# tianhao-stan-wu/LLA-MPC

Measured on AMD Instinct MI355X. Metric: model-rollouts/sec (N_models x H steps) per control tick; wall-clock per plan() call, higher is better.
Workload: dtype f64

## Files before the change

### lla-mpc_amd/csrc/final_dev.hpp

```cpp
#pragma once
#include "dev_stamps.hpp"
#include "dev_wave.hpp"
#include "lookback_dev.hpp"

namespace llampc {

__device__ __forceinline__ bool ent_less(const Ent& x, const Ent& y) {
  return less_nan_last(x.v, x.i, y.v, y.i);
}

template <typename E>
__device__ __forceinline__ E merge_path_at(const E* A, const E* B, int K, int k) {
  int lo = 0, hi = k;
  while (lo < hi) {
    const int i = (lo + hi) >> 1;
    if (less_nan_last(A[i].v, A[i].i, B[k - i - 1].v, B[k - i - 1].i)) lo = i + 1;
    else hi = i;
  }
  const int i = lo, j = k - lo;
  return (less_nan_last(A[i].v, A[i].i, B[j].v, B[j].i)) ? A[i] : B[j];
}

template <typename E>
__device__ __forceinline__ E* tree_merge(E* buf0, E* buf1, int L, int K) {
  E* src = buf0;
  E* dst = buf1;
  while (L > 1) {
    const int P = (L + 1) >> 1;
    for (int t = threadIdx.x; t < P * K; t += blockDim.x) {
      const int p = t / K, k = t - p * K;
      const E* A = src + (size_t)(2 * p) * K;
      dst[t] = (2 * p + 1 < L) ? merge_path_at(A, A + K, K, k) : A[k];
    }
    __syncthreads();
    E* tmp = src;
    src = dst;
    dst = tmp;
    L = P;
  }
  return src;
}

struct CtlSel {
  uint64_t* tag;
  uint32_t seq;
  uint32_t* ids;
  double* dr;
  double* df;
  double* xv;
  int32_t* xlate;
};

template <int SEL = 0>
__device__ __forceinline__ void lb_final(const FinalLaunch& f, unsigned char* smem, const CtlSel* cs = nullptr) {
  STAMP(0);
  const int tid = threadIdx.x;
  const int L = f.nb_lb;
  const int La = f.nb_lb * kWaves;
  const int K = f.K, M = L * K;
  uint64_t* thr = reinterpret_cast<uint64_t*>(smem + kScratchBytes);
  uint64_t* key = thr + 2;
  double* val = reinterpret_cast<double*>(key + M);
  uint64_t* hk = reinterpret_cast<uint64_t*>(val + M);
  uint64_t* ck = hk + L;
  Ent* am = reinterpret_cast<Ent*>(ck + M);
  uint32_t* id = reinterpret_cast<uint32_t*>(am + La);
  uint32_t* hid = id + M;
  uint32_t* cid = hid + L;
  int* ce = reinterpret_cast<int*>(cid + M);
  int* top = ce + M;
  int* cnt = top + LLAMPC_KMAX;
  auto local = [&](int64_t gi) { return gi == kNoIndex ? kNoLocal : (uint32_t)(gi - f.goff); };
  for (int e = tid; e < M; e += kBlock) {
    const double v = ld_wt(&f.tk_val[e]);
    const uint32_t l = local(ld_wt(&f.tk_idx[e]));
    const uint64_t k = l == kNoLocal ? ~0ull : order_key(v);
    const uint32_t i = l == kNoLocal ? kNoModelId + (uint32_t)e : l;
    key[e] = k;
    val[e] = v;
    id[e] = i;
    if (e % K == 0) {
      hk[e / K] = k;
      hid[e / K] = i;
    }
  }
  for (int b = tid; b < La; b += kBlock) am[b] = Ent{ld_wt(&f.am_val[b]), ld_wt(&f.am_idx[b])};
  if (tid == 0) {
    *cnt = 0;
    thr[0] = ~0ull;
    thr[1] = 0xFFFFFFFFull;
  }
  __syncthreads();
  STAMP(1);
  auto lt = [](uint64_t ka, uint32_t ia, uint64_t kb, uint32_t ib) {
    return (int)(ka < kb) | ((int)(ka == kb) & (int)(ia < ib));
  };
  if (L >= K) {
    for (int h = tid; h < L; h += kBlock) {
      const uint64_t mk = hk[h];
      const uint32_t mi = hid[h];
      int r = 0;
#pragma unroll 8
      for (int j = 0; j < L; ++j) r += lt(hk[j], hid[j], mk, mi);
      if (r == K - 1) {
        thr[0] = mk;
        thr[1] = mi;
      }
    }
    __syncthreads();
  }
  STAMP(6);
  const uint64_t tk = thr[0];
  const uint32_t ti = (uint32_t)thr[1];
  for (int e = tid; e < M; e += kBlock) {
    const uint64_t k = key[e];
    const uint32_t i = id[e];
    if (!lt(tk, ti, k, i)) {
      const int slot = atomicAdd(cnt, 1);
      ck[slot] = k;
      cid[slot] = i;
      ce[slot] = e;
    }
  }
  __syncthreads();
  STAMP(7);
  const int c = *cnt;
  for (int q = tid; q < c; q += kBlock) {
    const uint64_t mk = ck[q];
    const uint32_t mi = cid[q];
    int r = 0;
#pragma unroll 8
    for (int j = 0; j < c; ++j) r += lt(ck[j], cid[j], mk, mi);
    if (r < K) top[r] = ce[q];
  }
  __syncthreads();
  if (tid >= 64) return;
  const int lane = tid;
  double v = f.nan_first ? __builtin_inf() : __builtin_nan("");
  uint32_t li = kNoLocal;
  for (int b = lane; b < La; b += 64) {
    const double bv = am[b].v;
    const uint32_t bl = local(am[b].i);
    const bool t = (int)(bl != kNoLocal) &
                   (int)(f.nan_first ? less_bf<1>(bv, bl, v, li) : less_bf<0>(bv, bl, v, li));
    v = t ? bv : v;
    li = t ? bl : li;
  }
  if (f.nan_first) wave_pick_nf(v, li);
  else wave_pick_nl(v, li);
  double kv = __builtin_nan("");
  uint32_t kl = kNoLocal;
  if (lane < K) {
    const int e = top[lane];
    kl = id[e] >= kNoModelId ? kNoLocal : id[e];
    kv = val[e];
  }
  STAMP(2);
  if constexpr (SEL == 2) {
    if (lane < K) {
      cs->ids[lane] = kl;
      cs->xv[lane] = kv;
    }
    if (lane == 0) {
      cs->ids[K] = li;
      cs->xv[K] = v;
    }
    return;
  }
  if constexpr (SEL == 1) {
    if (lane < K) {
      cs->ids[lane] = kl;
      st_wt(&cs->tag[lane], tag_word(cs->seq, kl));
    }
    if (lane == 0) {
      cs->ids[K] = li;
      st_wt(&cs->tag[K], tag_word(cs->seq, li));
    }
  }
  llampc_plan_out* o = f.out;
  if (lane < LLAMPC_KMAX) {
    const int k = lane;
    if (k < K && kl != kNoLocal) {
      st_wt(&o->topk[k], f.goff + (int64_t)kl);
      st_wt(&o->topk_val[k], kv);
      st_wt(&o->topk_Df[k], f.params[2 * f.n + kl]);
      st_wt(&o->topk_Dr[k], f.params[5 * f.n + kl]);
    } else {
      const double nan = __builtin_nan("");
      st_wt(&o->topk[k], (int64_t)-1);
      st_wt(&o->topk_val[k], nan);
      st_wt(&o->topk_Df[k], nan);
      st_wt(&o->topk_Dr[k], nan);
    }
  }
  if (lane == 0) {
    st_wt(&o->lb_best, li == kNoLocal ? (int64_t)-1 : f.goff + (int64_t)li);
    st_wt(&o->lb_best_val, li == kNoLocal ? __builtin_nan("") : v);
  }
  if constexpr (SEL == 1) {
    if (lane < K) {
      const bool have = kl != kNoLocal;
      cs->dr[lane] = have ? f.params[5 * f.n + kl] : __builtin_nan("");
      cs->df[lane] = have ? f.params[2 * f.n + kl] : __builtin_nan("");
    }
  }
}

__device__ __forceinline__ void final_write(const FinalLaunch& f, bool lb, int64_t sel, bool owned,
                                            int32_t kcand, double kcost, int32_t scand,
                                            double scost, double lav, int64_t lai, int nf,
                                            int status = 0) {
  const int tid = threadIdx.x;
  llampc_plan_out* o = f.out;
  const double nan = __builtin_nan("");
  if (tid < LLAMPC_KMAX) {
    const int k = tid;
    if (!lb) {
      st_wt(&o->topk[k], (int64_t)-1);
      st_wt(&o->topk_val[k], nan);
      st_wt(&o->topk_Df[k], nan);
      st_wt(&o->topk_Dr[k], nan);
    }
    st_wt(&o->topk_cand[k], kcand);
    st_wt(&o->topk_cost[k], kcost);
  }
  if (tid == 0) {
    if (!lb) {
      st_wt(&o->lb_best, (int64_t)-1);
      st_wt(&o->lb_best_val, nan);
    }
    st_wt(&o->window_count, f.window_count);
    st_wt(&o->window_full, f.full);
    st_wt(&o->K, f.K);
    st_wt(&o->n_nonfinite, nf);
    st_wt(&o->status, status);
    st_wt(&o->sel_model, sel);
    st_wt(&o->sel_owned, (int32_t)owned);
    st_wt(&o->sel_cand, scand);
    st_wt(&o->sel_cost, scost);
    const bool la_ok = f.do_la && lai != kNoIndex;
    st_wt(&o->la_best_model, la_ok ? lai / f.C : (int64_t)-1);
    st_wt(&o->la_best_cand, la_ok ? (int32_t)(lai % f.C) : (int32_t)-1);
    st_wt(&o->la_best_cost, la_ok ? lav : nan);
    __hip_atomic_store(&f.tickets[0], 0u, __ATOMIC_RELAXED, __HIP_MEMORY_SCOPE_AGENT);
    __hip_atomic_store(&f.tickets[1], 0u, __ATOMIC_RELAXED, __HIP_MEMORY_SCOPE_AGENT);
    if (f.wq) __hip_atomic_store(f.wq, (uint64_t)0, __ATOMIC_RELAXED, __HIP_MEMORY_SCOPE_AGENT);
  }
  if (f.host_tag) {
    __threadfence_system();
    __syncthreads();
    if (tid == 0) __hip_atomic_store(f.host_tag, f.host_seq, __ATOMIC_RELAXED, __HIP_MEMORY_SCOPE_SYSTEM);
  }
  STAMP(5);
#ifdef LLAMPC_STAMPS
  if (tid == 0) g_stamp_launch++;
#endif
}

__device__ __forceinline__ void final_select(const FinalLaunch& f, const Scratch& sc) {
  STAMP(3);
  const int tid = threadIdx.x;
  llampc_plan_out* o = f.out;
  const bool lb = f.do_lb && f.full;
  const int64_t idk = (lb && tid < LLAMPC_KMAX) ? ld_wt(&o->topk[tid]) : -1;
  const int64_t lbi = (tid == 0 && lb) ? ld_wt(&o->lb_best) : -1;
  const int64_t sel = lbi >= 0 ? lbi : f.current_model;
  const bool owned = sel >= f.goff && sel < f.goff + f.n;
  const bool have = lb && tid < LLAMPC_KMAX && idk >= 0 && f.do_la;
  int32_t kcand = -1, scand = -1;
  double kcost = __builtin_nan(""), scost = __builtin_nan("");
  if (have) {
    kcand = ld_wt(&f.best_cand[idk - f.goff]);
    kcost = ld_wt(&f.best_cost[idk - f.goff]);
  }
  if (tid == 0 && owned && f.do_la) {
    scand = ld_wt(&f.best_cand[sel - f.goff]);
    scost = ld_wt(&f.best_cost[sel - f.goff]);
  }
  double lav = __builtin_nan("");
  int64_t lai = kNoIndex;
  int nf = 0;
  if (f.do_la) {
    for (int b = tid; b < f.nb_la; b += kBlock) {
      nf += ld_wt(&f.pnf[b]);
      const int64_t pi = ld_wt(&f.pidx[b]);
      const double pv = ld_wt(&f.pv[b]);
      const bool t = (int)(pi != kNoIndex) & (int)less_bf<0>(pv, pi, lav, lai);
      lav = t ? pv : lav;
      lai = t ? pi : lai;
    }
    wave_pick_nl64(lav, lai);
    nf = wave_sum(nf);
    if ((tid & 63) == 0) {
      sc.sv[4 + (tid >> 6)] = lav;
      sc.si[4 + (tid >> 6)] = lai;
      sc.sn[tid >> 6] = nf;
    }
    __syncthreads();
    lav = sc.sv[4];
    lai = sc.si[4];
    nf = sc.sn[0];
#pragma unroll
    for (int w = 1; w < kWaves; ++w) {
      const bool t = (int)(sc.si[4 + w] != kNoIndex) & (int)less_bf<0>(sc.sv[4 + w], sc.si[4 + w], lav, lai);
      lav = t ? sc.sv[4 + w] : lav;
      lai = t ? sc.si[4 + w] : lai;
      nf += sc.sn[w];
    }
  }
  STAMP(4);
  final_write(f, lb, sel, owned, kcand, kcost, scand, scost, lav, lai, nf);
}

constexpr int kPollTimeoutStatus = LLAMPC_STATUS_POLL_TIMEOUT;
__device__ __forceinline__ void final_poll(const FinalLaunch& f, const Scratch& sc) {
  STAMP(3);
  const int tid = threadIdx.x;
  llampc_plan_out* o = f.out;
  const bool lb = f.do_lb && f.full;
  const int64_t idk = (lb && tid < LLAMPC_KMAX) ? ld_wt(&o->topk[tid]) : -1;
  const int64_t lbi = (tid == 0 && lb) ? ld_wt(&o->lb_best) : -1;
  const int64_t sel = lbi >= 0 ? lbi : f.current_model;
  const bool owned = sel >= f.goff && sel < f.goff + f.n;
  const int64_t mk = (lb && tid < LLAMPC_KMAX && idk >= 0) ? idk - f.goff : -1;
  const int64_t ms = (tid == 0 && owned) ? sel - f.goff : -1;
  const int nbt = (f.nb_la + kBlock - 1) / kBlock;
  uint64_t kw[3] = {0, 0, 0}, sw[3] = {0, 0, 0};
  double lav = __builtin_nan("");
  int64_t lai = kNoIndex;
  int nf = 0;
  int status = 0;
  const uint64_t t0 = __builtin_amdgcn_s_memrealtime();
  const uint64_t bound = (uint64_t)(uint32_t)f.poll << 16;
  bool late = false;
  if (mk >= 0) {
    for (;;) {
#pragma unroll
      for (int w = 0; w < 3; ++w) kw[w] = ld_wt(&f.la_tag[w * f.n + mk]);
      if ((int)tag_ok(kw[0], f.seq) & (int)tag_ok(kw[1], f.seq) & (int)tag_ok(kw[2], f.seq)) break;
      if (__builtin_amdgcn_s_memrealtime() - t0 > bound) { late = true; break; }
    }
  }
  if (ms >= 0) {
    for (;;) {
#pragma unroll
      for (int w = 0; w < 3; ++w) sw[w] = ld_wt(&f.la_tag[w * f.n + ms]);
      if ((int)tag_ok(sw[0], f.seq) & (int)tag_ok(sw[1], f.seq) & (int)tag_ok(sw[2], f.seq)) break;
      if (__builtin_amdgcn_s_memrealtime() - t0 > bound) { late = true; break; }
    }
  }
  for (int j = 0; j < nbt; ++j) {
    const int b = tid + j * kBlock;
    if (b < f.nb_la) {
      uint64_t r[5];
      for (;;) {
#pragma unroll
        for (int w = 0; w < 5; ++w) r[w] = ld_wt(&f.blk_tag[5 * (int64_t)b + w]);
        if ((int)tag_ok(r[0], f.seq) & (int)tag_ok(r[1], f.seq) & (int)tag_ok(r[2], f.seq) &
            (int)tag_ok(r[3], f.seq) & (int)tag_ok(r[4], f.seq))
          break;
        if (__builtin_amdgcn_s_memrealtime() - t0 > bound) { late = true; break; }
      }
      const double pv = __longlong_as_double((long long)join_words(r[0], r[1]));
      const int64_t pi = (int64_t)join_words(r[2], r[3]);
      nf += (int)(uint32_t)r[4];
      const bool t = (int)(pi != kNoIndex) & (int)less_bf<0>(pv, pi, lav, lai);
      lav = t ? pv : lav;
      lai = t ? pi : lai;
    }
  }
  unsigned char* late_w = reinterpret_cast<unsigned char*>(sc.sv) + kLateOff;
  const int wlate = __any((int)late);
  int32_t kcand = -1, scand = -1;
  double kcost = __builtin_nan(""), scost = __builtin_nan("");
  if (mk >= 0 && f.do_la) {
    kcost = __longlong_as_double((long long)join_words(kw[0], kw[1]));
    kcand = (int32_t)(uint32_t)kw[2];
  }
  if (ms >= 0 && f.do_la) {
    scost = __longlong_as_double((long long)join_words(sw[0], sw[1]));
    scand = (int32_t)(uint32_t)sw[2];
  }
  wave_pick_nl64(lav, lai);
  nf = wave_sum(nf);
  if ((tid & 63) == 0) {
    sc.sv[4 + (tid >> 6)] = lav;
    sc.si[4 + (tid >> 6)] = lai;
    sc.sn[tid >> 6] = nf;
    late_w[tid >> 6] = (unsigned char)wlate;
  }
  __syncthreads();
  lav = sc.sv[4];
  lai = sc.si[4];
  nf = sc.sn[0];
  int anyl = late_w[0];
#pragma unroll
  for (int w = 1; w < kWaves; ++w) {
    const bool t = (int)(sc.si[4 + w] != kNoIndex) & (int)less_bf<0>(sc.sv[4 + w], sc.si[4 + w], lav, lai);
    lav = t ? sc.sv[4 + w] : lav;
    lai = t ? sc.si[4 + w] : lai;
    nf += sc.sn[w];
    anyl |= late_w[w];
  }
  if (anyl) status = kPollTimeoutStatus;
  STAMP(4);
  final_write(f, lb, sel, owned, kcand, kcost, scand, scost, lav, lai, nf, status);
}

}
```

### lla-mpc_amd/csrc/plan_dev.hpp

```cpp
#pragma once
#include "final_dev.hpp"
#include "lookahead_dev.hpp"
#include "lookback_dev.hpp"
#include "peer_dev.hpp"

namespace llampc {

template <int INTEG, bool STAGE, int LPM, int XM, bool PX = false, int WQ = 0, bool CORR = false>
__device__ __forceinline__ void plan_body(const LookbackLaunch& lb, const LookaheadLaunch& la,
                                          const FinalLaunch& fin, int G, int cpl,
                                          const double* hp = nullptr, double cw = 0.0) {
  extern __shared__ __attribute__((aligned(16))) unsigned char smem[];
  const Scratch sc(smem);
  int* flag = reinterpret_cast<int*>(smem + kFlagOff);
  const bool is_lb = (int)blockIdx.x < fin.nb_lb;
  const int lb_blk = (int)blockIdx.x, la_blk = (int)blockIdx.x - fin.nb_lb;
  if constexpr (wq_threads(WQ) > kBlock) {
    if (is_lb && threadIdx.x >= kBlock) return;
  }
  if (is_lb) {
    lookback_block(lb, lb_blk, sc);
    if (!ticket_last(&fin.tickets[0], (unsigned)fin.nb_lb, flag)) return;
    if (fin.full) {
      lb_final(fin, smem);
      if (fin.host_tag) __threadfence_system();
    }
    if (fin.poll) {
      __syncthreads();
      final_poll(fin, sc);
      if constexpr (PX) peer_finish(fin, smem);
      return;
    }
  } else {
    if constexpr (CORR) lookahead_block<INTEG, STAGE, LPM, XM, WQ, true>(la, la_blk, G, cpl, smem, sc, hp, cw);
    else lookahead_block<INTEG, STAGE, LPM, XM, WQ>(la, la_blk, G, cpl, smem, sc);
    if (fin.poll) return;
    if constexpr (wq_threads(WQ) > kBlock) {
      if (threadIdx.x >= kBlock) return;
    }
  }
  const unsigned expected = (unsigned)fin.nb_la + (fin.nb_lb > 0 ? 1u : 0u);
  if (!ticket_last(&fin.tickets[1], expected, flag)) return;
  final_select(fin, sc);
  if constexpr (PX) peer_finish(fin, smem);
}

constexpr int kArgLa = sizeof(LookbackLaunch), kArgFin = kArgLa + sizeof(LookaheadLaunch);
constexpr int kArgG = kArgFin + sizeof(FinalLaunch), kPlanArgBytes = kArgG + 2 * sizeof(int);
static_assert(sizeof(LookbackLaunch) % 8 == 0 && sizeof(LookaheadLaunch) % 8 == 0 && sizeof(FinalLaunch) % 8 == 0,
              "plan kernel arguments: no padding between the launch structs");

template <int INTEG, bool STAGE, int LPM, int XM, bool PX = false, int WQ = 0>
__global__ __launch_bounds__(wq_threads(WQ)) void plan_kernel(LookbackLaunch lb, LookaheadLaunch la,
                                                      FinalLaunch fin, int G, int cpl) {
  if constexpr (XM || WQ) {
    plan_body<INTEG, STAGE, LPM, XM, PX, WQ>(lb, la, fin, G, cpl);
  } else {
    const KernargPtr kp = touch_kernargs<kPlanArgBytes>();
    plan_body<INTEG, STAGE, LPM, XM, PX, WQ>(kernarg_at<LookbackLaunch>(kp, 0), kernarg_at<LookaheadLaunch>(kp, kArgLa),
                                             kernarg_at<FinalLaunch>(kp, kArgFin), kernarg_at<int>(kp, kArgG),
                                             kernarg_at<int>(kp, kArgG + 4));
  }
}

template <int LPM>
__global__ __launch_bounds__(kBlock) void plan_kernel_inl(LookbackLaunch, LookaheadLaunch, FinalLaunch, int, int,
                                                          InlinePack pk) {
  const KernargPtr kp = touch_kernargs<kPlanArgBytes>();
  LookbackLaunch lb = kernarg_at<LookbackLaunch>(kp, 0);
  LookaheadLaunch la = kernarg_at<LookaheadLaunch>(kp, kArgLa);
  const double* v = pk.v;
  lb.x_prev = v;
  lb.u_prev = v + 6;
  lb.x_now = v + 8;
  la.x0 = v + 8;
  la.uprev = v + 14;
  la.xref = v + 16;
  la.U = v + 16 + 2 * (la.H + 1);
  plan_body<0, true, LPM, 0>(lb, la, kernarg_at<FinalLaunch>(kp, kArgFin), kernarg_at<int>(kp, kArgG),
                             kernarg_at<int>(kp, kArgG + 4));
}

template <int INTEG, bool STAGE, int LPM>
__global__ __launch_bounds__(kBlock) void plan_kernel_corr(LookbackLaunch, LookaheadLaunch, FinalLaunch, int, int,
                                                           PlanCorridor cor) {
  const KernargPtr kp = touch_kernargs<kPlanArgBytes>();
  plan_body<INTEG, STAGE, LPM, 0, false, 0, true>(kernarg_at<LookbackLaunch>(kp, 0), kernarg_at<LookaheadLaunch>(kp, kArgLa),
                                                  kernarg_at<FinalLaunch>(kp, kArgFin), kernarg_at<int>(kp, kArgG),
                                                  kernarg_at<int>(kp, kArgG + 4), cor.hp, cor.weight);
}

template <int INTEG, bool STAGE, int PX, int WQ>
static void launch_plan_wq(const LookbackLaunch& lb, const LookaheadLaunch& la, const FinalLaunch& f,
                           int G, int cpl, size_t lds, hipStream_t s) {
  allow_lds(plan_kernel<INTEG, STAGE, 1, 0, PX, WQ>);
  hipLaunchKernelGGL((plan_kernel<INTEG, STAGE, 1, 0, PX, WQ>), dim3(f.nb_lb + f.nb_la), dim3(wq_threads(WQ)),
                     lds, s, lb, la, f, G, cpl);
}

template <int INTEG, bool STAGE, int LPM>
static void launch_plan_t(const LookbackLaunch& lb, const LookaheadLaunch& la, const FinalLaunch& f,
                          int G, int cpl, size_t lds, hipStream_t s, int wq = 0) {
  if constexpr (INTEG == LLAMPC_RK4 && LPM == 1) {
    if (wq) {
      if constexpr (STAGE) {
        if (wq == 2) {
          if (f.px_G) launch_plan_wq<INTEG, STAGE, 1, 2>(lb, la, f, G, cpl, lds, s);
          else launch_plan_wq<INTEG, STAGE, 0, 2>(lb, la, f, G, cpl, lds, s);
          return;
        }
      }
      if (f.px_G) launch_plan_wq<INTEG, STAGE, 1, 1>(lb, la, f, G, cpl, lds, s);
      else launch_plan_wq<INTEG, STAGE, 0, 1>(lb, la, f, G, cpl, lds, s);
      return;
    }
  }
  if constexpr (INTEG == LLAMPC_RK4) {
    if (f.px_G) {
      allow_lds(plan_kernel<INTEG, STAGE, LPM, 0, true>);
      hipLaunchKernelGGL((plan_kernel<INTEG, STAGE, LPM, 0, true>), dim3(f.nb_lb + f.nb_la), dim3(kBlock), lds,
                         s, lb, la, f, G, cpl);
      return;
    }
  }
  if (la.xref_mode == LLAMPC_XREF_RACELINE) {
    allow_lds(plan_kernel<INTEG, STAGE, LPM, 1>);
    hipLaunchKernelGGL((plan_kernel<INTEG, STAGE, LPM, 1>), dim3(f.nb_lb + f.nb_la), dim3(kBlock), lds, s,
                       lb, la, f, G, cpl);
  } else {
    allow_lds(plan_kernel<INTEG, STAGE, LPM, 0>);
    hipLaunchKernelGGL((plan_kernel<INTEG, STAGE, LPM, 0>), dim3(f.nb_lb + f.nb_la), dim3(kBlock), lds, s,
                       lb, la, f, G, cpl);
  }
}

template <int LPM>
static void launch_plan_inl(const LookbackLaunch& lb, const LookaheadLaunch& la, const FinalLaunch& f,
                            int G, int cpl, size_t lds, hipStream_t s, const InlinePack& pk) {
  allow_lds(plan_kernel_inl<LPM>);
  hipLaunchKernelGGL((plan_kernel_inl<LPM>), dim3(f.nb_lb + f.nb_la), dim3(kBlock), lds, s, lb, la, f,
                     G, cpl, pk);
}

template <int INTEG, int LPM>
void launch_plan_group(const LookbackLaunch& lb, const LookaheadLaunch& la, const FinalLaunch& f, int G,
                       int cpl, bool stage, size_t lds, hipStream_t s, int wq) {
  if (stage) launch_plan_t<INTEG, true, LPM>(lb, la, f, G, cpl, lds, s, wq);
  else launch_plan_t<INTEG, false, LPM>(lb, la, f, G, cpl, lds, s, wq);
}

template <int LPM>
void launch_plan_inline_group(const LookbackLaunch& lb, const LookaheadLaunch& la, const FinalLaunch& f,
                              int G, int cpl, size_t lds, hipStream_t s, const InlinePack& pk) {
  launch_plan_inl<LPM>(lb, la, f, G, cpl, lds, s, pk);
}

template <int INTEG, bool STAGE, int LPM>
static void launch_plan_corr(const LookbackLaunch& lb, const LookaheadLaunch& la, const FinalLaunch& f, int G,
                             int cpl, size_t lds, hipStream_t s, const PlanCorridor& cor) {
  allow_lds(plan_kernel_corr<INTEG, STAGE, LPM>);
  hipLaunchKernelGGL((plan_kernel_corr<INTEG, STAGE, LPM>), dim3(f.nb_lb + f.nb_la), dim3(kBlock), lds, s, lb, la, f,
                     G, cpl, cor);
}

template <int INTEG, int LPM>
void launch_plan_corridor_group(const LookbackLaunch& lb, const LookaheadLaunch& la, const FinalLaunch& f, int G,
                                int cpl, bool stage, size_t lds, hipStream_t s, const PlanCorridor& cor) {
  if (stage) launch_plan_corr<INTEG, true, LPM>(lb, la, f, G, cpl, lds, s, cor);
  else launch_plan_corr<INTEG, false, LPM>(lb, la, f, G, cpl, lds, s, cor);
}

}
```

### lla-mpc_amd/csrc/plan_track_dev.hpp

```cpp
#pragma once
#include "corridor_block_dev.hpp"
#include "ctl_door_dev.hpp"
#include "plan_dev.hpp"

namespace llampc {

#ifdef LLAMPC_STAMPS
static __device__ unsigned long long g_trk_ph[1024][8];
#define TRK_STAMP(slot)                                                                              \
  do {                                                                                               \
    if (threadIdx.x == 0 && blockIdx.x < 1024) g_trk_ph[blockIdx.x][slot] = __builtin_amdgcn_s_memrealtime(); \
  } while (0)
#else
#define TRK_STAMP(slot) LLAMPC_NO_STAMP
#endif

__device__ __forceinline__ void track_corridor_block(const PlanTrack& k, int kk, unsigned char* smem) {
  TRK_STAMP(0);
  const bool valid = k.path_ok != 0 && *k.valid_rd != 0;
  const double nan = __builtin_nan("");
  double px = nan, py = nan, p0x = nan, p0y = nan;
  if (valid) {
    px = k.path_rd[kk];
    py = k.path_rd[kPlanPathStride + kk];
    if (kk == 1) {
      p0x = k.path_rd[0];
      p0y = k.path_rd[kPlanPathStride];
    }
  }
  auto emit = [&](const double* row, double theta) {
    uint64_t* w = k.hp_tag + 12 * (size_t)(kk - 1);
#pragma unroll
    for (int i = 0; i < 6; ++i) {
      const uint64_t b = (uint64_t)__double_as_longlong(row[i]);
      st_wt(&w[2 * i], tag_word(k.seq, (uint32_t)(b >> 32)));
      st_wt(&w[2 * i + 1], tag_word(k.seq, (uint32_t)b));
    }
    double* d = k.dbg;
    d[kk] = px;
    d[kPlanPathStride + kk] = py;
    if (kk == 1) {
      d[0] = p0x;
      d[kPlanPathStride] = p0y;
      *k.dbg_valid = valid;
    }
    double* dh = d + 2 * kPlanPathStride + 6 * (size_t)(kk - 1);
#pragma unroll
    for (int i = 0; i < 6; ++i) dh[i] = row[i];
    d[2 * kPlanPathStride + 6 * LLAMPC_HMAX + (kk - 1)] = theta;
    TRK_STAMP(1);
  };
  if (valid) {
    corridor_block(k.trk, smem, px, py, k.hw, emit);
  } else if (threadIdx.x == 0) {
    const double inf = __builtin_inf();
    const double row[6] = {0.0, 0.0, inf, 0.0, 0.0, inf};
    emit(row, nan);
  }
}

__device__ __forceinline__ int track_poll_hp(const PlanTrack& k, int H, double* shp) {
  uint32_t* hp32 = reinterpret_cast<uint32_t*>(shp);
  int any = 0;
  for (int e = threadIdx.x; e < 12 * H; e += kBlock) {
    int late = 0;
    const uint32_t v = poll_tag(k.hp_tag, e, k.seq, k.poll, late);
    hp32[(e & ~1) | ((e & 1) ^ 1)] = late ? 0u : v;
    any |= late;
  }
  return any;
}

__device__ __forceinline__ void track_stage_write(const LookaheadLaunch& a, double* o, double ua, double dl, double sd,
                                                  double cd, double p0, double p1, const FusedK& fq0) {
  const double d0 = ua - p0, d1 = dl - p1;
  const FusedIn fi = fused_in(fq0, Input{ua, dl, sd, cd});
  o[0] = fi.F0;
  o[1] = fi.F1;
  o[2] = fi.hmsd;
  o[3] = fi.hmcd;
  o[4] = fi.c5a;
  o[5] = dl;
  o[6] = act_term(a.cost, d0, d1);
  o[7] = (!a.cost.enforce || input_feasible(a.cost, ua, dl, d0, d1)) ? 1.0 : 0.0;
}

__device__ __forceinline__ void track_pin_consts(CostK& q, VehK& veh, double& Ts) {
  for (int m = 0; m < 4; ++m) {
    pin_vgpr(q.Q[m]);
    pin_vgpr(q.R[m]);
    pin_vgpr(q.P[m]);
  }
  for (int m = 0; m < 2; ++m) {
    pin_vgpr(q.umin[m]);
    pin_vgpr(q.umax[m]);
    pin_vgpr(q.dmax[m]);
  }
  pin_vgpr(veh.lf);
  pin_vgpr(veh.lr);
  pin_vgpr(veh.mass);
  pin_vgpr(veh.inv_mass);
  pin_vgpr(veh.inv_Iz);
  pin_vgpr(veh.Cm1);
  pin_vgpr(veh.Cm2);
  pin_vgpr(veh.Cr0);
  pin_vgpr(veh.Cr2);
  pin_vgpr(Ts);
}

template <int LPM>
__device__ __forceinline__ void track_model_setup(const VehK& veh, const Tire& t, int sub, double Ts, StageK& sk,
                                                  FusedK& fq) {
  constexpr bool kScaled = scaled_yaw(LPM);
  sk = make_stage<LPM>(veh, t, sub, Ts, Ts * veh.inv_mass);
  if (kScaled) sk.ch[0].lw = sk.ch[0].lw / Ts;
  if (kScaled && LPM == 1) sk.ch[1].lw = sk.ch[1].lw / Ts;
  if (kScaled && LPM == 4 && sub >= 2) {
    sk.ch[0].lw = 0.0;
    sk.ch[0].sg = 0.0;
    sk.ch[0].B = 0.0;
    sk.ch[0].nsB = 0.0;
    sk.Bfw = 0.0;
  }
  fq = make_fused(veh, sk, Ts, kScaled, LPM == 4);
}

template <bool STAGE, int LPM>
__device__ __forceinline__ void track_lookahead_block(const LookaheadLaunch& a, int blk, int G, int cpl,
                                                      unsigned char* smem, const Scratch& sc, const PlanTrack& trk) {
  LA_STAMP(blk, 0);
  TRK_STAMP(0);
  constexpr int BT = kBlock;
  double* sx = reinterpret_cast<double*>(smem + kScratchBytes);
  double* su = sx + 2 * (a.H + 1);
  const int H = a.H, C = a.C;
  double* shp = su + (STAGE ? kStageW * C * H : 0);
  const int sub = threadIdx.x % LPM;
  const int cl = threadIdx.x / LPM;
  const int g = cl & (G - 1);
  const int64_t n = (int64_t)blk * (kBlock / (G * LPM)) + cl / G;
  const bool live = n < a.n;
  Tire t{};
  if (live) t = load_tire(a.params, a.n, n);
  double x0[6];
  CostK q = a.cost;
  VehK veh = a.veh;
  double Ts = a.Ts;
  StageK sk;
  FusedK fq;
  fm::FmK K0;
  double up0, up1;
  {
    const int CH = C * H, tid = (int)threadIdx.x;
    uint32_t zoff;
    asm volatile("v_mov_b32 %0, 0" : "=v"(zoff));
    const double* gx0 = a.x0 + zoff;
    const double* gup = a.uprev + zoff;
    double xv[6];
#pragma unroll
    for (int m = 0; m < 6; ++m) xv[m] = gx0[m];
    const double uv0 = gup[0], uv1 = gup[1];
    const int ex = tid < H ? tid : H;
    const double xr0 = a.xref[ex], xr1 = a.xref[(H + 1) + ex];
    auto stage_load = [&](int e, double& ua, double& dl, double& p0, double& p1) {
      const int ec = e < CH ? e : CH - 1, ep = ec > 0 ? ec - 1 : 0;
      ua = a.U[2 * ec];
      dl = a.U[2 * ec + 1];
      p0 = a.U[2 * ep];
      p1 = a.U[2 * ep + 1];
    };
    double sua = 0.0, sdl = 0.0, sp0 = 0.0, sp1 = 0.0;
    if (STAGE) stage_load(tid, sua, sdl, sp0, sp1);
    K0 = load_la_consts<0, LPM>();
    track_pin_consts(q, veh, Ts);
    track_model_setup<LPM>(veh, t, sub, Ts, sk, fq);
    for (int e = tid; e <= H; e += BT) {
      sx[2 * e] = e == tid ? xr0 : a.xref[e];
      sx[2 * e + 1] = e == tid ? xr1 : a.xref[(H + 1) + e];
    }
#pragma unroll
    for (int m = 0; m < 6; ++m) x0[m] = readfirstlane_d(xv[m]);
    up0 = readfirstlane_d(uv0);
    up1 = readfirstlane_d(uv1);
    if (STAGE) {
      const FusedK fq0 = make_fused(a.veh, make_stage<1>(a.veh, Tire{}, 0), a.Ts, scaled_yaw(LPM));
      auto stage_elem = [&](int e, double ua, double dl, double p0, double p1) {
        const int c = C == 1 ? 0 : e / H, k = e - c * H;
        double sd, cd;
        if (fm::sincos_fast_ok(dl)) fm::sincos_fast(dl, &sd, &cd, K0);
        else LL_SINCOS(dl, &sd, &cd);
        track_stage_write(a, su + kStageW * (k * C + c), ua, dl, sd, cd, k ? p0 : uv0, k ? p1 : uv1, fq0);
      };
      if (tid < CH) stage_elem(tid, sua, sdl, sp0, sp1);
      constexpr int kStageBatch = 4;
      for (int base = tid + BT; base < CH; base += kStageBatch * BT) {
        double ua[kStageBatch], dl[kStageBatch], p0[kStageBatch], p1[kStageBatch];
#pragma unroll
        for (int j = 0; j < kStageBatch; ++j) stage_load(base + j * BT, ua[j], dl[j], p0[j], p1[j]);
#pragma unroll
        for (int j = 0; j < kStageBatch; ++j)
          if (base + j * BT < CH) stage_elem(base + j * BT, ua[j], dl[j], p0[j], p1[j]);
      }
    }
    asm volatile("" ::"v"(xr0), "v"(xr1), "v"(sua), "v"(sdl), "v"(sp0), "v"(sp1));
    TRK_STAMP(1);
    if (track_poll_hp(trk, H, shp)) {
      st_wt(trk.late, trk.seq);
      asm volatile("s_waitcnt vmcnt(0)" ::: "memory");
    }
    TRK_STAMP(2);
    __syncthreads();
  }

  double bv = __builtin_nan("");
  int64_t bc = kNoIndex;
  int nf = 0;
  LA_STAMP(blk, 1);
  constexpr unsigned kRF = STAGE ? kRStage : 0u;
  const double cw = trk.weight;
  if (live) {
    const fm::FmK K = K0;
    for (int j = 0; j < cpl; ++j) {
      const int c = g + j * G;
      if (c >= C) break;
      bool bad = false;
      double J = rollout<0, LPM, kRF | kRFast | kRCorr>(a, c, n, x0, sx, su, veh, t, sk, q, Ts, up0, up1, K, fq, bad,
                                                        nullptr, nullptr, nullptr, 0, nullptr, shp, cw);
      if (LPM == 2) {
        const int bi = bad;
        bad = __builtin_amdgcn_mov_dpp(bi, kPair0, 0xF, 0xF, false) |
              __builtin_amdgcn_mov_dpp(bi, kPair1, 0xF, 0xF, false);
      } else if (LPM == 4) {
        int bi = bad;
        bi |= __builtin_amdgcn_mov_dpp(bi, kQuadX1, 0xF, 0xF, false);
        bi |= __builtin_amdgcn_mov_dpp(bi, kQuadX2, 0xF, 0xF, false);
        bad = bi;
      }
      if (__builtin_expect(__any(bad), 0)) {
        bool unused = false;
        if (bad) J = rollout<0, LPM, kRF | kRCorr>(a, c, n, x0, sx, su, veh, t, sk, q, Ts, up0, up1, K, fq, unused,
                                                   nullptr, nullptr, nullptr, 0, nullptr, shp, cw);
      }
      if (sub == 0) {
        if (a.cost_out) a.cost_out[n * C + c] = J;
        nf += !isfinite(J);
      }
      if (less_nan_last(J, c, bv, bc)) {
        bv = J;
        bc = c;
      }
    }
  }
  LA_STAMP(blk, 2);
  TRK_STAMP(3);
  const int span = G * LPM;
  for (int off = (span < 64 ? span : 64) >> 1; off >= LPM; off >>= 1) {
    const double ov = __shfl_xor(bv, off, 64);
    const int64_t oc = __shfl_xor(bc, off, 64);
    if (less_nan_last(ov, oc, bv, bc)) {
      bv = ov;
      bc = oc;
    }
  }
  int par = 0;
  if (span > 64) {
    double* sv = sc.sv + 4 * par;
    int64_t* si = sc.si + 4 * par;
    par ^= 1;
    if ((threadIdx.x & 63) == 0) {
      sv[threadIdx.x >> 6] = bv;
      si[threadIdx.x >> 6] = bc;
    }
    __syncthreads();
    const int w0 = (int)(threadIdx.x / span) * (span / 64);
    bv = sv[w0];
    bc = si[w0];
    for (int k = 1; k < span / 64; ++k) {
      if (less_nan_last(sv[w0 + k], si[w0 + k], bv, bc)) {
        bv = sv[w0 + k];
        bc = si[w0 + k];
      }
    }
  }
  if (live && g == 0 && sub == 0) {
    if (a.poll) {
      st_wt(&a.la_tag[n], tag_word(a.seq, (uint32_t)(__double_as_longlong(bv) >> 32)));
      st_wt(&a.la_tag[a.n + n], tag_word(a.seq, (uint32_t)__double_as_longlong(bv)));
      st_wt(&a.la_tag[2 * a.n + n], tag_word(a.seq, (uint32_t)(int32_t)bc));
    } else {
      st_wt(&a.best_cand[n], (int32_t)bc);
      st_wt(&a.best_cost[n], bv);
    }
  }
  const int64_t key = (live && bc != kNoIndex && g == 0 && sub == 0) ? (a.goff + n) * C + bc : kNoIndex;
  la_publish(a, blk, sc, par, (key == kNoIndex) ? __builtin_nan("") : bv, key, nf);
  LA_STAMP(blk, 3);
  TRK_STAMP(4);
}

template <bool STAGE, int LPM>
__device__ __forceinline__ void track_path_update(const LookaheadLaunch& a, const FinalLaunch& f, const PlanTrack& trk,
                                                  unsigned char* smem) {
  const int tid = threadIdx.x, H = a.H;
  double* sx = reinterpret_cast<double*>(smem + kScratchBytes);
  double* su = sx + 2 * (H + 1);
  double* shp = su + kStageW * H;
  double* ppos = shp + 6 * H;
  double* sx0 = ppos + 2 * (H + 1);
  double* pcost = sx0 + 6;
  int64_t* psel = reinterpret_cast<int64_t*>(pcost + 1);
  int* pint = reinterpret_cast<int*>(psel + 1);
  __syncthreads();
  if (tid == 0) {
    psel[0] = ld_wt(&f.out->sel_model);
    pint[0] = ld_wt(&f.out->sel_cand);
    pint[1] = ld_wt(&f.out->sel_owned);
    pint[2] = 0;
    *pcost = __builtin_nan("");
  }
  __syncthreads();
  const int64_t sel = psel[0];
  const int cand = pint[0];
  const bool can = pint[1] == 1 && cand >= 0 && cand < a.C && sel >= a.goff && sel < a.goff + a.n;
  if (!can) {
    if (tid == 0) {
      *trk.cost_wr = __builtin_nan("");
      *trk.valid_wr = 0;
    }
    return;
  }
  LookaheadLaunch a1 = a;
  a1.C = 1;
  a1.U = a.U + 2 * (size_t)cand * H;
  const fm::FmK K0 = load_la_consts<0, LPM>();
  for (int e = tid; e <= H; e += kBlock) {
    sx[2 * e] = a.xref[e];
    sx[2 * e + 1] = a.xref[(H + 1) + e];
  }
  if (tid < 6) sx0[tid] = a.x0[tid];
  const double uv0 = a.uprev[0], uv1 = a.uprev[1];
  if (STAGE) {
    const FusedK fq0 = make_fused(a.veh, make_stage<1>(a.veh, Tire{}, 0), a.Ts, scaled_yaw(LPM));
    for (int k = tid; k < H; k += kBlock) {
      const double ua = a1.U[2 * k], dl = a1.U[2 * k + 1];
      const double p0 = k ? a1.U[2 * k - 2] : uv0, p1 = k ? a1.U[2 * k - 1] : uv1;
      double sd, cd;
      if (fm::sincos_fast_ok(dl)) fm::sincos_fast(dl, &sd, &cd, K0);
      else LL_SINCOS(dl, &sd, &cd);
      track_stage_write(a, su + kStageW * k, ua, dl, sd, cd, p0, p1, fq0);
    }
  }
  (void)track_poll_hp(trk, H, shp);
  __syncthreads();
  if (tid < LPM) {
    const int sub = tid;
    const Tire t = load_tire(a.params, a.n, sel - a.goff);
    CostK q = a.cost;
    VehK veh = a.veh;
    double Ts = a.Ts;
    track_pin_consts(q, veh, Ts);
    StageK sk;
    FusedK fq;
    track_model_setup<LPM>(veh, t, sub, Ts, sk, fq);
    double x0[6];
#pragma unroll
    for (int m = 0; m < 6; ++m) x0[m] = sx0[m];
    constexpr unsigned kRF = STAGE ? kRStage : 0u;
    double* dp = sub == 0 ? ppos : nullptr;
    bool bad = false, unused = false;
    double Jw = rollout<0, LPM, kRF | kRFast | kRCorr | kRPos>(a1, 0, sel - a.goff, x0, sx, su, veh, t, sk, q, Ts, uv0, uv1,
                                                               K0, fq, bad, nullptr, nullptr, dp, H + 1, nullptr, shp,
                                                               trk.weight);
    merge_bad<LPM>(bad);
    if (bad)
      Jw = rollout<0, LPM, kRF | kRCorr | kRPos>(a1, 0, sel - a.goff, x0, sx, su, veh, t, sk, q, Ts, uv0, uv1, K0, fq,
                                                 unused, nullptr, nullptr, dp, H + 1, nullptr, shp, trk.weight);
    if (sub == 0) {
      *pcost = Jw;
      pint[2] = (int)(fabs(Jw) <= __DBL_MAX__);
    }
  }
  __syncthreads();
  if (tid < 64) {
    bool ok = pint[2] != 0;
    for (int e = tid; e < 2 * (H + 1); e += 64) {
      const int row = e / (H + 1), j = e - row * (H + 1);
      const double v = ppos[row * (H + 1) + ctl_path_index(j, H)];
      ok = ok && fabs(v) <= __DBL_MAX__;
      trk.path_wr[row * kPlanPathStride + j] = v;
    }
    const int all = __all(ok);
    if (tid == 0) {
      *trk.cost_wr = *pcost;
      *trk.valid_wr = all;
    }
  }
  TRK_STAMP(7);
}

__device__ __forceinline__ void track_finish(const FinalLaunch& f, const PlanTrack& trk) {
  if (threadIdx.x == 0 && ld_wt(trk.late) == trk.seq) st_wt(&f.out->status, (int32_t)kPollTimeoutStatus);
  if (f.host_tag) {
    __threadfence_system();
    __syncthreads();
    if (threadIdx.x == 0) __hip_atomic_store(f.host_tag, f.host_seq, __ATOMIC_RELAXED, __HIP_MEMORY_SCOPE_SYSTEM);
  }
}

template <bool STAGE, int LPM>
__device__ __forceinline__ void plan_track_body(const LookbackLaunch& lb, const LookaheadLaunch& la,
                                                const FinalLaunch& fin, int G, int cpl, const PlanTrack& trk) {
  extern __shared__ __attribute__((aligned(16))) unsigned char smem[];
  const Scratch sc(smem);
  int* flag = reinterpret_cast<int*>(smem + kFlagOff);
  const int blk = (int)blockIdx.x, H = la.H;
  if (blk >= fin.nb_lb && blk < fin.nb_lb + H) {
    track_corridor_block(trk, blk - fin.nb_lb + 1, smem);
    return;
  }
  FinalLaunch fq = fin;
  fq.host_tag = nullptr;
  const bool is_lb = blk < fin.nb_lb;
  if (is_lb) {
    lookback_block(lb, blk, sc);
    if (!ticket_last(&fin.tickets[0], (unsigned)fin.nb_lb, flag)) return;
    if (fin.full) {
      lb_final(fin, smem);
      if (fin.host_tag) __threadfence_system();
    }
    if (fin.poll) {
      __syncthreads();
      TRK_STAMP(5);
      final_poll(fq, sc);
      track_finish(fin, trk);
      TRK_STAMP(6);
      track_path_update<STAGE, LPM>(la, fin, trk, smem);
      return;
    }
  } else {
    track_lookahead_block<STAGE, LPM>(la, blk - fin.nb_lb - H, G, cpl, smem, sc, trk);
    if (fin.poll) return;
  }
  const unsigned expected = (unsigned)fin.nb_la + (fin.nb_lb > 0 ? 1u : 0u);
  if (!ticket_last(&fin.tickets[1], expected, flag)) return;
  TRK_STAMP(5);
  final_select(fq, sc);
  track_finish(fin, trk);
  TRK_STAMP(6);
  track_path_update<STAGE, LPM>(la, fin, trk, smem);
}

constexpr int kArgTrack = kPlanArgBytes;
static_assert(kPlanArgBytes % alignof(PlanTrack) == 0, "the PlanTrack lies right behind (G, cpl)");

template <bool STAGE, int LPM>
__global__ __launch_bounds__(kBlock) void plan_kernel_track(LookbackLaunch, LookaheadLaunch, FinalLaunch, int, int,
                                                            PlanTrack) {
  const KernargPtr kp = touch_kernargs<kPlanArgBytes>();
  plan_track_body<STAGE, LPM>(kernarg_at<LookbackLaunch>(kp, 0), kernarg_at<LookaheadLaunch>(kp, kArgLa),
                              kernarg_at<FinalLaunch>(kp, kArgFin), kernarg_at<int>(kp, kArgG),
                              kernarg_at<int>(kp, kArgG + 4), kernarg_at<PlanTrack>(kp, kArgTrack));
}

template <bool STAGE, int LPM>
static void launch_plan_track_t(const LookbackLaunch& lb, const LookaheadLaunch& la, const FinalLaunch& f, int G,
                                int cpl, size_t lds, hipStream_t s, const PlanTrack& trk) {
  allow_lds(plan_kernel_track<STAGE, LPM>);
  hipLaunchKernelGGL((plan_kernel_track<STAGE, LPM>), dim3(f.nb_lb + la.H + f.nb_la), dim3(kBlock), lds, s, lb, la, f,
                     G, cpl, trk);
}

}
```

Baseline: 9.276 billion.

## Keep lookback selection in registers and poll all tags concurrently in final_poll

The lookback final stage now returns its top-K and best selection in registers instead of writing them to the output struct and reading them back in the poll path. That removes a global round trip and a block barrier. The poll loop now issues model-tag and block-tag loads together in one combined spin loop, rather than waiting on each sequentially. The output record is written once at the end. This adds register pressure and more complex loop logic, and changes when partial outputs become visible.

New measurement: 9.128 billion. 1.6% lower.

```diff
diff --git a/lla-mpc_amd/csrc/final_dev.hpp b/lla-mpc_amd/csrc/final_dev.hpp
--- a/lla-mpc_amd/csrc/final_dev.hpp
+++ b/lla-mpc_amd/csrc/final_dev.hpp
@@ -51,8 +51,18 @@
   int32_t* xlate;
 };
 
-template <int SEL = 0>
-__device__ __forceinline__ void lb_final(const FinalLaunch& f, unsigned char* smem, const CtlSel* cs = nullptr) {
+struct LbSel {
+  uint32_t kl;
+  double kv;
+  uint32_t li;
+  double v;
+};
+__device__ __forceinline__ LbSel no_sel() { return LbSel{kNoLocal, __builtin_nan(""), kNoLocal, __builtin_nan("")}; }
+
+template <int SEL = 0, bool REC = true>
+__device__ __forceinline__ void lb_final(const FinalLaunch& f, unsigned char* smem, const CtlSel* cs = nullptr,
+                                         LbSel* sel = nullptr) {
+  static_assert(REC || SEL == 0, "the controller's selections write their record here");
   STAMP(0);
   const int tid = threadIdx.x;
   const int L = f.nb_lb;
@@ -156,6 +166,10 @@
     kv = val[e];
   }
   STAMP(2);
+  if constexpr (!REC) {
+    *sel = LbSel{kl, kv, li, v};
+    return;
+  }
   if constexpr (SEL == 2) {
     if (lane < K) {
       cs->ids[lane] = kl;
@@ -206,8 +220,19 @@
   }
 }
 
-__device__ __forceinline__ void final_write(const FinalLaunch& f, bool lb, int64_t sel, bool owned,
-                                            int32_t kcand, double kcost, int32_t scand,
+struct LbHalf {
+  int64_t topk;
+  double val, Df, Dr;
+  int64_t best;
+  double best_val;
+};
+__device__ __forceinline__ LbHalf no_half() {
+  const double nan = __builtin_nan("");
+  return LbHalf{-1, nan, nan, nan, -1, nan};
+}
+
+__device__ __forceinline__ void final_write(const FinalLaunch& f, bool put_lb, const LbHalf& h, int64_t sel,
+                                            bool owned, int32_t kcand, double kcost, int32_t scand,
                                             double scost, double lav, int64_t lai, int nf,
                                             int status = 0) {
   const int tid = threadIdx.x;
@@ -215,19 +240,19 @@
   const double nan = __builtin_nan("");
   if (tid < LLAMPC_KMAX) {
     const int k = tid;
-    if (!lb) {
-      st_wt(&o->topk[k], (int64_t)-1);
-      st_wt(&o->topk_val[k], nan);
-      st_wt(&o->topk_Df[k], nan);
-      st_wt(&o->topk_Dr[k], nan);
+    if (put_lb) {
+      st_wt(&o->topk[k], h.topk);
+      st_wt(&o->topk_val[k], h.val);
+      st_wt(&o->topk_Df[k], h.Df);
+      st_wt(&o->topk_Dr[k], h.Dr);
     }
     st_wt(&o->topk_cand[k], kcand);
     st_wt(&o->topk_cost[k], kcost);
   }
   if (tid == 0) {
-    if (!lb) {
-      st_wt(&o->lb_best, (int64_t)-1);
-      st_wt(&o->lb_best_val, nan);
+    if (put_lb) {
+      st_wt(&o->lb_best, h.best);
+      st_wt(&o->lb_best_val, h.best_val);
     }
     st_wt(&o->window_count, f.window_count);
     st_wt(&o->window_full, f.full);
@@ -239,8 +264,11 @@
     st_wt(&o->sel_cand, scand);
     st_wt(&o->sel_cost, scost);
     const bool la_ok = f.do_la && lai != kNoIndex;
-    st_wt(&o->la_best_model, la_ok ? lai / f.C : (int64_t)-1);
-    st_wt(&o->la_best_cand, la_ok ? (int32_t)(lai % f.C) : (int32_t)-1);
+    int64_t bm = -1;
+    int32_t bc = -1;
+    if (la_ok) split_key(lai, f.C, bm, bc);
+    st_wt(&o->la_best_model, bm);
+    st_wt(&o->la_best_cand, bc);
     st_wt(&o->la_best_cost, la_ok ? lav : nan);
     __hip_atomic_store(&f.tickets[0], 0u, __ATOMIC_RELAXED, __HIP_MEMORY_SCOPE_AGENT);
     __hip_atomic_store(&f.tickets[1], 0u, __ATOMIC_RELAXED, __HIP_MEMORY_SCOPE_AGENT);
@@ -309,23 +337,24 @@
     }
   }
   STAMP(4);
-  final_write(f, lb, sel, owned, kcand, kcost, scand, scost, lav, lai, nf);
+  final_write(f, !lb, no_half(), sel, owned, kcand, kcost, scand, scost, lav, lai, nf);
 }
 
 constexpr int kPollTimeoutStatus = LLAMPC_STATUS_POLL_TIMEOUT;
-__device__ __forceinline__ void final_poll(const FinalLaunch& f, const Scratch& sc) {
+__device__ __forceinline__ void final_poll(const FinalLaunch& f, const Scratch& sc, const LbSel& s) {
   STAMP(3);
   const int tid = threadIdx.x;
-  llampc_plan_out* o = f.out;
   const bool lb = f.do_lb && f.full;
-  const int64_t idk = (lb && tid < LLAMPC_KMAX) ? ld_wt(&o->topk[tid]) : -1;
-  const int64_t lbi = (tid == 0 && lb) ? ld_wt(&o->lb_best) : -1;
-  const int64_t sel = lbi >= 0 ? lbi : f.current_model;
+  const bool w0 = tid < 64;
+  const uint32_t kl = (lb && w0 && tid < f.K) ? s.kl : kNoLocal;
+  const uint32_t li = (lb && w0) ? s.li : kNoLocal;
+  const int64_t sel = li != kNoLocal ? f.goff + (int64_t)li : f.current_model;
   const bool owned = sel >= f.goff && sel < f.goff + f.n;
-  const int64_t mk = (lb && tid < LLAMPC_KMAX && idk >= 0) ? idk - f.goff : -1;
-  const int64_t ms = (tid == 0 && owned) ? sel - f.goff : -1;
-  const int nbt = (f.nb_la + kBlock - 1) / kBlock;
-  uint64_t kw[3] = {0, 0, 0}, sw[3] = {0, 0, 0};
+  const bool hk = kl != kNoLocal, hs = tid == 0 && owned;
+  const int64_t mk = hk ? (int64_t)kl : 0;
+  const int64_t ms = hs ? sel - f.goff : 0;
+  const double df = f.params[2 * f.n + mk], dr = f.params[5 * f.n + mk];
+  uint64_t kw[3] = {0, 0, 0}, sw[3] = {0, 0, 0}, r[5] = {0, 0, 0, 0, 0};
   double lav = __builtin_nan("");
   int64_t lai = kNoIndex;
   int nf = 0;
@@ -333,51 +362,70 @@
   const uint64_t t0 = __builtin_amdgcn_s_memrealtime();
   const uint64_t bound = (uint64_t)(uint32_t)f.poll << 16;
   bool late = false;
-  if (mk >= 0) {
-    for (;;) {
+  int b = (tid + kBlock - 64) & (kBlock - 1);
+  const int nb = f.nb_la;
+  const bool wrec = b - (tid & 63) < nb;
+  typedef const __attribute__((address_space(1))) uint64_t* GWords;
+  uint32_t seq = f.seq;
+  uint64_t la_u = (uint64_t)f.la_tag, blk_u = (uint64_t)f.blk_tag;
+  int64_t n = f.n;
+  asm volatile("" : "+s"(seq), "+s"(la_u), "+s"(blk_u), "+s"(n));
+  const GWords la_tag = (GWords)la_u, blk_tag = (GWords)blk_u;
+  auto issue = [&]() {
+    const int64_t bb = b < nb ? b : 0;
+    if (w0) {
 #pragma unroll
-      for (int w = 0; w < 3; ++w) kw[w] = ld_wt(&f.la_tag[w * f.n + mk]);
-      if ((int)tag_ok(kw[0], f.seq) & (int)tag_ok(kw[1], f.seq) & (int)tag_ok(kw[2], f.seq)) break;
-      if (__builtin_amdgcn_s_memrealtime() - t0 > bound) { late = true; break; }
-    }
-  }
-  if (ms >= 0) {
-    for (;;) {
+      for (int w = 0; w < 3; ++w) kw[w] = __hip_atomic_load(&la_tag[w * n + mk], __ATOMIC_RELAXED, __HIP_MEMORY_SCOPE_AGENT);
 #pragma unroll
-      for (int w = 0; w < 3; ++w) sw[w] = ld_wt(&f.la_tag[w * f.n + ms]);
-      if ((int)tag_ok(sw[0], f.seq) & (int)tag_ok(sw[1], f.seq) & (int)tag_ok(sw[2], f.seq)) break;
-      if (__builtin_amdgcn_s_memrealtime() - t0 > bound) { late = true; break; }
-    }
-  }
-  for (int j = 0; j < nbt; ++j) {
-    const int b = tid + j * kBlock;
-    if (b < f.nb_la) {
-      uint64_t r[5];
-      for (;;) {
+      for (int w = 0; w < 3; ++w) sw[w] = __hip_atomic_load(&la_tag[w * n + ms], __ATOMIC_RELAXED, __HIP_MEMORY_SCOPE_AGENT);
+    }
+    if (wrec) {
 #pragma unroll
-        for (int w = 0; w < 5; ++w) r[w] = ld_wt(&f.blk_tag[5 * (int64_t)b + w]);
-        if ((int)tag_ok(r[0], f.seq) & (int)tag_ok(r[1], f.seq) & (int)tag_ok(r[2], f.seq) &
-            (int)tag_ok(r[3], f.seq) & (int)tag_ok(r[4], f.seq))
-          break;
-        if (__builtin_amdgcn_s_memrealtime() - t0 > bound) { late = true; break; }
-      }
+      for (int w = 0; w < 5; ++w) r[w] = __hip_atomic_load(&blk_tag[5 * bb + w], __ATOMIC_RELAXED, __HIP_MEMORY_SCOPE_AGENT);
+    }
+  };
+  issue();
+  for (;;) {
+    int ok = 1;
+    if (w0) {
+      const int okk = (int)tag_ok(kw[0], seq) & (int)tag_ok(kw[1], seq) & (int)tag_ok(kw[2], seq);
+      const int oks = (int)tag_ok(sw[0], seq) & (int)tag_ok(sw[1], seq) & (int)tag_ok(sw[2], seq);
+      ok = ((int)!hk | okk) & ((int)!hs | oks);
+    }
+    if (b < nb && ((int)tag_ok(r[0], seq) & (int)tag_ok(r[1], seq) & (int)tag_ok(r[2], seq) &
+                   (int)tag_ok(r[3], seq) & (int)tag_ok(r[4], seq))) {
       const double pv = __longlong_as_double((long long)join_words(r[0], r[1]));
       const int64_t pi = (int64_t)join_words(r[2], r[3]);
       nf += (int)(uint32_t)r[4];
       const bool t = (int)(pi != kNoIndex) & (int)less_bf<0>(pv, pi, lav, lai);
       lav = t ? pv : lav;
       lai = t ? pi : lai;
-    }
+      b += kBlock;
+    }
+    if (ok & (int)(b >= nb)) break;
+    if (__builtin_amdgcn_s_memrealtime() - t0 > bound) { late = true; break; }
+    issue();
+  }
+  LbHalf h = no_half();
+  if (hk) {
+    h.topk = f.goff + (int64_t)kl;
+    h.val = s.kv;
+    h.Df = df;
+    h.Dr = dr;
+  }
+  if (tid == 0 && li != kNoLocal) {
+    h.best = f.goff + (int64_t)li;
+    h.best_val = s.v;
   }
   unsigned char* late_w = reinterpret_cast<unsigned char*>(sc.sv) + kLateOff;
   const int wlate = __any((int)late);
   int32_t kcand = -1, scand = -1;
   double kcost = __builtin_nan(""), scost = __builtin_nan("");
-  if (mk >= 0 && f.do_la) {
+  if (hk && f.do_la) {
     kcost = __longlong_as_double((long long)join_words(kw[0], kw[1]));
     kcand = (int32_t)(uint32_t)kw[2];
   }
-  if (ms >= 0 && f.do_la) {
+  if (hs && f.do_la) {
     scost = __longlong_as_double((long long)join_words(sw[0], sw[1]));
     scand = (int32_t)(uint32_t)sw[2];
   }
@@ -404,7 +452,7 @@
   }
   if (anyl) status = kPollTimeoutStatus;
   STAMP(4);
-  final_write(f, lb, sel, owned, kcand, kcost, scand, scost, lav, lai, nf, status);
-}
-
-}
+  final_write(f, true, h, sel, owned, kcand, kcost, scand, scost, lav, lai, nf, status);
+}
+
+}
diff --git a/lla-mpc_amd/csrc/plan_dev.hpp b/lla-mpc_amd/csrc/plan_dev.hpp
--- a/lla-mpc_amd/csrc/plan_dev.hpp
+++ b/lla-mpc_amd/csrc/plan_dev.hpp
@@ -21,15 +21,16 @@
   if (is_lb) {
     lookback_block(lb, lb_blk, sc);
     if (!ticket_last(&fin.tickets[0], (unsigned)fin.nb_lb, flag)) return;
+    if (fin.poll) {
+      LbSel sel = no_sel();
+      if (fin.full) lb_final<0, false>(fin, smem, nullptr, &sel);
+      final_poll(fin, sc, sel);
+      if constexpr (PX) peer_finish(fin, smem);
+      return;
+    }
     if (fin.full) {
       lb_final(fin, smem);
       if (fin.host_tag) __threadfence_system();
-    }
-    if (fin.poll) {
-      __syncthreads();
-      final_poll(fin, sc);
-      if constexpr (PX) peer_finish(fin, smem);
-      return;
     }
   } else {
     if constexpr (CORR) lookahead_block<INTEG, STAGE, LPM, XM, WQ, true>(la, la_blk, G, cpl, smem, sc, hp, cw);
diff --git a/lla-mpc_amd/csrc/plan_track_dev.hpp b/lla-mpc_amd/csrc/plan_track_dev.hpp
--- a/lla-mpc_amd/csrc/plan_track_dev.hpp
+++ b/lla-mpc_amd/csrc/plan_track_dev.hpp
@@ -424,14 +424,11 @@
   if (is_lb) {
     lookback_block(lb, blk, sc);
     if (!ticket_last(&fin.tickets[0], (unsigned)fin.nb_lb, flag)) return;
-    if (fin.full) {
-      lb_final(fin, smem);
-      if (fin.host_tag) __threadfence_system();
-    }
     if (fin.poll) {
-      __syncthreads();
+      LbSel sel = no_sel();
+      if (fin.full) lb_final<0, false>(fin, smem, nullptr, &sel);
       TRK_STAMP(5);
-      final_poll(fq, sc);
+      final_poll(fq, sc, sel);
       track_finish(fin, trk);
       TRK_STAMP(6);
       track_path_update<STAGE, LPM>(la, fin, trk, smem);
```
